# facebookresearch/AVID-CMA

Measured on AMD Instinct MI355X. Metric: clips/sec (video+audio fwd+bwd+NCE+Adam), higher is better.
Workload: dtype f32 (bf16x3 MFMA)

## Files before the change

### avid-cma_amd/avid_hip/lib.py

```python
from __future__ import annotations

import ctypes as C
import os
import subprocess


import torch

_HERE = os.path.dirname(os.path.abspath(__file__))
_PKG = os.path.dirname(_HERE)
LIB_PATH = os.environ.get("AVID_HIP_LIB") or os.path.join(_HERE, "libavid_hip.so")

AVID_OK = 0


class BnBwdFuse(C.Structure):
    _fields_ = [("x", C.c_void_p), ("scale", C.c_void_p), ("shift", C.c_void_p), ("mean", C.c_void_p),
                ("invstd", C.c_void_p), ("relu", C.c_int32), ("partials", C.c_void_p)]


class InAffine(C.Structure):
    _fields_ = [("scale", C.c_void_p), ("shift", C.c_void_p), ("relu", C.c_int32)]


# ... 79 lines not shown
    "avid_timing_enable": (_i, [_i]),
    "avid_timing_report": (_i, [C.c_char_p, _sz]),
    "avid_conv_fwd_workspace_bytes": (_sz, [_dp]),
    "avid_conv_fwd_stats_rows": (_i, [_dp]),
    "avid_conv_fwd": (_i, [_dp, _vp, _vp, _vp, _vp, _vp, _i, _vp, _vp, _vp, _sz, _vp]),
    "avid_conv_takes_in_affine": (_i, [_dp]),
    "avid_conv_fwd_in": (_i, [_dp, _vp, _vp, _vp, _vp, _vp, _vp, _i, _vp, _vp, _vp, _sz, _vp]),
    "avid_debug_in_affine_launches": (C.c_longlong, [_i]),
    "avid_conv_takes_out_affine": (_i, [_dp]),
    "avid_conv_fwd_out": (_i, [_dp, _vp, _vp, _vp, _vp, _vp, _vp, _i, _vp, _vp, _vp, _vp, _sz, _vp]),
    "avid_debug_out_affine_launches": (C.c_longlong, []),
    "avid_conv_dgrad_workspace_bytes": (_sz, [_dp]),
    "avid_conv_dgrad_bn_rows": (_i, [_dp]),
    "avid_conv_dgrad": (_i, [_dp, _vp, _vp, _vp, _vp, _vp, _vp, _vp, _vp, _vp, _sz, _vp]),
    "avid_weight_transpose_batched": (_i, [_i, _vp, _i64, _vp]),
    "avid_weight_transform": (_i, [_vp, _vp]),
    "avid_conv_wgrad_workspace_bytes": (_sz, [_dp]),
    "avid_conv_wgrad": (_i, [_dp, _vp, _vp, _vp, _vp, _sz, _vp]),
    "avid_conv_wgrad_in": (_i, [_dp, _vp, _vp, _vp, _vp, _vp, _sz, _vp]),
    "avid_conv_wgrad_groupable": (_i, [_dp]),
    "avid_conv_wgrad_group_workspace_bytes": (_sz, [_i, C.POINTER(WgradItem)]),
    "avid_conv_wgrad_group": (_i, [_i, C.POINTER(WgradItem), _vp, _sz, _vp]),
    "avid_conv_kernel_name": (_i, [_dp, _i, C.c_char_p, _i]),
    "avid_conv_uses_wino": (_i, [_dp, _i]),
    "avid_conv_uses_split": (_i, [_dp, _i]),
    "avid_conv_split_bytes": (_sz, [_dp]),
    "avid_debug_presplit_launches": (C.c_longlong, []),
    "avid_wino_configure": (_i, [_i, _i64, _i]),
    "avid_wino2_configure": (_i, [_i]),
    "avid_wino2_pre_configure": (_i, [_i]),
    "avid_wgrad_pre_configure": (_i, [_i]),
    "avid_stem_fwd_pre_configure": (_i, [_i]),
    "avid_tconv_configure": (_i, [_i]),
    "avid_set_cu_budget": (_i, [_i]),
    "avid_cu_budget": (_i, []),
    "avid_bn_workspace_bytes": (_sz, [_i64, _i]),
    "avid_bn_fwd_train": (_i, [_i64, _i, _vp, _vp, _vp, _vp, _vp, _f, _f, _i, _vp, _vp, _vp, _vp, _vp, _vp, _vp, _i, _vp, _sz, _vp]),
    "avid_bn_fwd_eval": (_i, [_i64, _i, _vp, _vp, _vp, _vp, _vp, _f, _i, _vp, _vp, _vp]),
    "avid_bn_eval_coeffs_batched": (_i, [_i, _vp, _vp]),
    "avid_bn_apply_eval": (_i, [_i64, _i, _vp, _vp, _vp, _i, _vp, _vp]),
    "avid_bn_relu_maxpool_fwd_eval": (_i, [_i, _i, _i, _i, _i, _vp, _vp, _vp, _vp, _vp]),
    "avid_bn_bwd": (_i, [_i64, _i, _vp, _vp, _vp, _vp, _vp, _vp, _vp, _i, _vp, _vp, _vp, _vp, _i, _i, _vp, _sz, _vp]),
    "avid_bn_relu_maxpool_fwd": (_i, [_i, _i, _i, _i, _i, _vp, _vp, _vp, _vp, _vp, _f, _f, _vp, _vp, _vp, _vp, _vp, _vp, _vp,
                                      _vp, _i, _vp, _sz, _vp]),
    "avid_bn_relu_maxpool_bwd": (_i, [_i, _i, _i, _i, _i, _vp, _vp, _vp, _vp, _vp, _vp, _vp, _vp, _vp, _vp, _vp, _vp, _sz,
                                      _vp]),
    "avid_clip_normalize": (_i, [_i, _i, _i, _i, _vp, C.POINTER(_f), C.POINTER(_f), _vp, _vp]),
    "avid_clip_augment_workspace_bytes": (_sz, [_i, C.POINTER(AugDesc), _i, _i, _i]),
    "avid_clip_augment": (_i, [_i, C.POINTER(AugDesc), _i, _i, _i, C.POINTER(_f), C.POINTER(_f), _vp, _vp, _sz, _vp]),
    "avid_logspec_basis_floats": (_sz, [_i]),
    "avid_logspec_basis": (_i, [_i, _vp, _vp]),
    "avid_logspec_workspace_bytes": (_sz, [_i, _i, _i]),
    "avid_logspec": (_i, [_i, _i, _vp, _i, _i, _i, _vp, _vp, _vp, _f, _vp, _vp, _sz, _vp]),
    "avid_maxpool_hw3s2_fwd": (_i, [_i, _i, _i, _i, _i, _vp, _vp, _vp, _vp]),
    "avid_maxpool_hw3s2_bwd": (_i, [_i, _i, _i, _i, _i, _vp, _vp, _vp, _vp]),
    "avid_global_maxpool_fwd": (_i, [_i, _i, _i, _vp, _vp, _vp, _vp]),
    "avid_global_maxpool_bwd": (_i, [_i, _i, _i, _vp, _vp, _vp, _vp]),
    "avid_relu_bwd": (_i, [_i64, _vp, _vp, _vp, _vp]),
    "avid_colsum": (_i, [_i64, _i, _vp, _vp, _vp]),
    "avid_l2norm_fwd": (_i, [_i, _i, _vp, _vp, _vp, _vp]),
    "avid_l2norm_bwd": (_i, [_i, _i, _vp, _vp, _vp, _vp, _vp]),
    "avid_alias_draw": (_i, [_i64, _i64, _vp, _vp, _i, _u64, _u64, _vp, _vp, _i64, _vp, _vp]),
    "avid_counter_add": (_i, [_vp, _u64, _vp]),
    "avid_dropout_fwd": (_i, [_i64, _i64, _f, _u64, _u64, _vp, _vp, _vp, _vp, _vp]),
    "avid_dropout_bwd": (_i, [_i64, _f, _vp, _vp, _vp, _vp]),
    "avid_cls_loss": (_i, [_i, _i, _i, _vp, _vp, _f, _vp, _vp, _vp, _vp, _vp, _vp]),
# ... 101 lines not shown
```

### avid-cma_amd/csrc/conv.hip

```cpp
#include <math.h>
#include <stdlib.h>

#include <atomic>
#include <type_traits>

#include "common.h"

namespace avid {

typedef unsigned int uintx4 __attribute__((ext_vector_type(4)));

struct ConvArgs {
  const float* __restrict__ src;
  const float* __restrict__ wk;
  int w_row, w_nrec;
  const float* __restrict__ addend;
  const float* __restrict__ bias;
  float* __restrict__ dst;
  float* __restrict__ part;
  int B, Ts, Hs, Ws, Cs;
  int Td, Hd, Wd, Cd;
  int kt, kh, kw;
  int st, sh, sw;
  int pt, ph, pw;
// ... 281 lines not shown

constexpr int EPI_ANY = 15;
#ifdef AVID_PK_TRACE
__device__ long long g_pk_trace[1024 * 64];
extern "C" int avid_debug_pk_trace(long long* host) {
  return (int)hipMemcpyFromSymbol(host, HIP_SYMBOL(g_pk_trace), sizeof(long long) * 1024 * 64);
}
#define PK_STAMP(idx) do { if (threadIdx.x == 0 && (idx) < 32) { g_pk_trace[blockIdx.x * 64 + (idx)] = wall_clock64(); g_pk_trace[blockIdx.x * 64 + 32 + (idx)] = clock64(); } } while (0)
#else
#define PK_STAMP(idx) do {} while (0)
#endif
#ifdef AVID_PK_FP32
constexpr bool PK_SPLIT = false;
#else
constexpr bool PK_SPLIT = true;
#endif
typedef __bf16 pk_bf16x8 __attribute__((ext_vector_type(8)));
typedef unsigned pk_uintx4 __attribute__((ext_vector_type(4)));
template <bool DOT = true>
__device__ __forceinline__ void pk_split8(const floatx4& v0, const floatx4& v1, pk_bf16x8& fh, pk_bf16x8& fm, pk_bf16x8& fl) {
  const float v[8] = {v0[0], v0[1], v0[2], v0[3], v1[0], v1[1], v1[2], v1[3]};
  unsigned h[4], m[4], l[4];
#pragma unroll
  for (int i = 0; i < 4; ++i) {
    if (DOT) split2_bf16_dot(v[2 * i], v[2 * i + 1], h[i], m[i], l[i]);
    else split2_bf16(v[2 * i], v[2 * i + 1], h[i], m[i], l[i]);
  }
  fh = __builtin_bit_cast(pk_bf16x8, pk_uintx4{h[0], h[1], h[2], h[3]});
  fm = __builtin_bit_cast(pk_bf16x8, pk_uintx4{m[0], m[1], m[2], m[3]});
  fl = __builtin_bit_cast(pk_bf16x8, pk_uintx4{l[0], l[1], l[2], l[3]});
}

constexpr int PK_BCH = 2 * 2 * 3 * 1024;
template <int WM, int WN, int TM, int TN, int MODE, bool STRIDED = false, int EPI = EPI_ANY, bool BS = false>
__global__ __launch_bounds__(WM * WN * 64, 2) void igemm_pk_kernel(const ConvArgs p) {
  static_assert(!STRIDED || MODE == 1, "parity classes are a dgrad construct");
  constexpr int NT = WM * WN * 64;
  constexpr int BM = WM * TM * 32, BN = WN * TN * 32;
  constexpr int RPP = NT / 8;
  constexpr int PA = BM / RPP, PB = BN / RPP;
  static_assert(BM % RPP == 0 && BN % RPP == 0, "tile rows must be a multiple of the staging pass");
  static_assert(!BS || (NT == 256 && (BN == 64 || BN == 128) && PK_SPLIT), "pre-split weights: the 4-wave tiles of the split-bf16 build");
  constexpr int BCH = (BN / 64) * PK_BCH;
  constexpr int PB3 = BCH / (NT * 16);
  constexpr bool ASWZ = BS && BN == 128;
  constexpr int ALD = ASWZ ? BK : LDK;
  constexpr int STAGE = BS ? BM * ALD + BCH / 4 : (BM + BN) * LDK;
  extern __shared__ __attribute__((aligned(16))) float smem[];
  typedef const ConvArgs __attribute__((address_space(4)))* KArgs;
  const KArgs kp = (KArgs)__builtin_amdgcn_kernarg_segment_ptr();
  const int tid = threadIdx.x, lane = tid & 63, wave = tid >> 6;
  const int wm = wave / WN, wn = wave % WN;
  const int lrow = tid >> 3, lcol = (tid & 7) * 4;
  const int h = lane >> 5, l31 = lane & 31;
  PK_STAMP(0);

  const int ntn = p.Cd / BN;
  const int G = gridDim.x;
  int slot_;
  if (p.pk_paired) {
    const int per = G >> 4;
    const int xcd = blockIdx.x & 7, pos = blockIdx.x >> 3;
    const int second = pos >= per ? 1 : 0;
    slot_ = second * (G >> 1) + xcd * per + (pos - second * per);
  } else {
    slot_ = (int)xcd_remap(blockIdx.x, G);
  }
  const int slot = __builtin_amdgcn_readfirstlane(slot_);
  const int ntaps = p.kt * p.kh * p.kw;
  const int cpt = p.Cs / BK;
  const int nk = ntaps * cpt;
  const int cs4 = p.Cs * 4;
  const int pix_per_b = p.Ts * p.Hs * p.Ws;
  const int pix_d = p.Td * p.Hd * p.Wd;
  const __amdgpu_buffer_rsrc_t rsB = __builtin_amdgcn_make_buffer_rsrc(
      BS ? const_cast<void*>(p.wsp) : (void*)p.wk, 0, BS ? p.wsp_nrec : p.w_nrec, 0x00020000);

  const int n_full = slot < p.pk_full ? (p.pk_full - slot + G - 1) / G : 0;
  int tslot = slot - p.pk_rot;
  tslot += tslot < 0 ? G : 0;
  const int nseg = n_full + (tslot < p.pk_tail_units ? 1 : 0);
// ... 49 lines not shown
      const int kps = (nkc + fc - 1) / fc;
      k0 = piece * kps < nkc ? piece * kps : nkc;
      k1 = k0 + kps < nkc ? k0 + kps : nkc;
      split = fc > 1 ? piece : -1;
    } else if (j < n_full) {
      tile = slot + j * G; k0 = 0; k1 = nk; split = -1;
    } else {
      int piece;
      if (p.pk_ws) {
        const int r = tslot / p.pk_ws, mt = tslot - r * p.pk_ws;
        const int nt = r / p.pk_f;
        piece = r - nt * p.pk_f;
        tile = p.pk_full + mt * ntn + nt;
      } else {
        tile = p.pk_full + tslot / p.pk_f;
        piece = tslot % p.pk_f;
      }
      split = p.pk_f > 1 ? piece : -1;
      k0 = piece * p.pk_kps;
      k1 = k0 + p.pk_kps < nk ? k0 + p.pk_kps : nk;
    }
  };

  int ld_seg = 0, ld_ks = 0, ld_kend = 0;
  int ld_dt = 0, ld_dh = 0, ld_dw = 0, ld_c0 = 0, ld_tap = 0;
  int ld_nh = p.kh, ld_nw = p.kw, ld_cls = 0;
  int ld_plo = 0, ld_phi = 0, ld_nrec = 0;
  int ld_soff_a = 0, ld_soff_b = 0;
  unsigned a_base[PA], a_mask[PA], a_cur[PA];
  unsigned b_off[PB];
  floatx4 va[PA], vb[PB];
  pk_uintx4 vb3[PB3];
  int ld_bnt = 0;

  auto range_mask = [](int lo, int hi, int k) -> unsigned {
    lo = lo < 0 ? 0 : lo;
    hi = hi > k - 1 ? k - 1 : hi;
    return hi >= lo ? (2u << hi) - (1u << lo) : 0u;
  };
  auto retap = [&]() {
    const int pixoff = ((ld_dt * p.Hs + ld_dh) * p.Ws + ld_dw) * cs4;
    const unsigned tap_off = (unsigned)(MODE == 0 ? pixoff : -pixoff);
    const unsigned sh_t = ld_dt, sh_h = 8 + ld_dh, sh_w = 16 + ld_dw;
#pragma unroll
    for (int i = 0; i < PA; ++i) {
      const unsigned okb = (a_mask[i] >> sh_t) & (a_mask[i] >> sh_h) & (a_mask[i] >> sh_w) & 1u;
      a_cur[i] = okb ? a_base[i] + tap_off : OOB;
    }
  };
  auto setup_tile = [&](int tile) {
    int c = 0, cT = p.Td, cH = p.Hd, cW = p.Wd, cM = p.M, cpix = pix_d, lt = tile;
    unsigned mgW = p.mgW, mgH = p.mgH, mgT = p.mgT;
    int shW = p.shW, shH = p.shH, shT = p.shT;
    int offt = p.pt, offh = p.ph, offw = p.pw, ndt = p.kt, ndh = p.kh, ndw = p.kw;
    if (STRIDED) {
      c = ld_cls;
      lt = tile - kp->cls_begin[c];
      cT = kp->cls_n[c][0]; cH = kp->cls_n[c][1]; cW = kp->cls_n[c][2];
      cpix = cT * cH * cW;
      cM = p.B * cpix;
      mgT = kp->cls_mg[c][0]; mgH = kp->cls_mg[c][1]; mgW = kp->cls_mg[c][2];
      shT = kp->cls_shf[c][0]; shH = kp->cls_shf[c][1]; shW = kp->cls_shf[c][2];
      offt = (kp->cls_p0[c][0] + p.pt - kp->cls_d0[c][0]) / p.st;
      offh = (kp->cls_p0[c][1] + p.ph - kp->cls_d0[c][1]) / p.sh;
      offw = (kp->cls_p0[c][2] + p.pw - kp->cls_d0[c][2]) / p.sw;
      ndt = kp->cls_nd[c][0]; ndh = kp->cls_nd[c][1]; ndw = kp->cls_nd[c][2];
// ... 33 lines not shown
        mh = range_mask(-h0, p.Hs - 1 - h0, p.kh);
        mw = range_mask(-w0, p.Ws - 1 - w0, p.kw);
      } else {
        t0 = td + offt; h0 = hd + offh; w0 = wd + offw;
        mt_ = range_mask(t0 - p.Ts + 1, t0, ndt);
        mh = range_mask(h0 - p.Hs + 1, h0, ndh);
        mw = range_mask(w0 - p.Ws + 1, w0, ndw);
      }
      dec_mask = ok ? (mt_ | (mh << 8) | (mw << 16)) : 0u;
      dec_base = (unsigned)((((b - b_lo) * p.Ts + t0) * p.Hs + h0) * p.Ws + w0) * cs4;
    }
#pragma unroll
    for (int i = 0; i < PA; ++i) {
      const int src = (lane & ~7) | i;
      a_mask[i] = (unsigned)__shfl((int)dec_mask, src, 64);
      a_base[i] = (unsigned)__shfl((int)dec_base, src, 64) + lcol * 4;
    }
#pragma unroll
    for (int i = 0; i < PB; ++i) b_off[i] = (unsigned)((n0 + lrow + RPP * i) * p.w_row + lcol) * 4;
    if (BS) ld_bnt = __builtin_amdgcn_readfirstlane(nt * BCH);
  };
  auto issue_loads = [&]() {
    const unsigned long long ptr = ((unsigned long long)(unsigned)__builtin_amdgcn_readfirstlane(ld_phi) << 32) |
                                   (unsigned)__builtin_amdgcn_readfirstlane(ld_plo);
    const __amdgpu_buffer_rsrc_t rsA = __builtin_amdgcn_make_buffer_rsrc(
        reinterpret_cast<void*>(ptr), 0, __builtin_amdgcn_readfirstlane(ld_nrec), 0x00020000);
    const int soff_a = __builtin_amdgcn_readfirstlane(ld_soff_a);
    const int soff_b = __builtin_amdgcn_readfirstlane(ld_soff_b);
#pragma unroll
    for (int i = 0; i < PA; ++i)
      va[i] = __builtin_bit_cast(floatx4, __builtin_amdgcn_raw_buffer_load_b128(rsA, a_cur[i], soff_a, 0));
    if (BS) {
      const int soff_b3 = __builtin_amdgcn_readfirstlane(ld_soff_b + ld_bnt);
#pragma unroll
      for (int i = 0; i < PB3; ++i)
        vb3[i] = __builtin_bit_cast(pk_uintx4, __builtin_amdgcn_raw_buffer_load_b128(rsB, (tid + NT * i) * 16, soff_b3, 0));
      return;
    }
#pragma unroll
    for (int i = 0; i < PB; ++i)
      vb[i] = __builtin_bit_cast(floatx4, __builtin_amdgcn_raw_buffer_load_b128(rsB, b_off[i], soff_b, 0));
  };
  const auto sgpr = [](int v) { return __builtin_amdgcn_readfirstlane(v); };
  auto set_tap = [&]() {
    if (STRIDED) {
      const int c = ld_cls;
      ld_tap = sgpr(((kp->cls_d0[c][0] + ld_dt * p.st) * p.kh + kp->cls_d0[c][1] + ld_dh * p.sh) * p.kw + kp->cls_d0[c][2] +
                    ld_dw * p.sw);
    } else {
      ld_tap = sgpr((ld_dt * p.kh + ld_dh) * p.kw + ld_dw);
    }
    ld_soff_a = sgpr(ld_c0 * 4);
    ld_soff_b = BS ? sgpr((ld_tap * cpt + ld_c0 / BK) * p.wsp_kstep) : sgpr((ld_tap * p.Cs + ld_c0) * 4);
  };
  auto setup_seg = [&](int j) {
    int tile, k0, k1, split;
    seg_info(j, tile, k0, k1, split);
    if (STRIDED) {
      while (k1 == k0 && j + 1 < nseg) seg_info(++j, tile, k0, k1, split);
      ld_seg = sgpr(k1 == k0 ? nseg : j);
      if (k1 == k0) return;
      ld_cls = sgpr(cls_of(tile));
      ld_nh = sgpr(kp->cls_nd[ld_cls][1]);
      ld_nw = sgpr(kp->cls_nd[ld_cls][2]);
    }
    ld_ks = sgpr(k0);
// ... 8 lines not shown
    setup_tile(tile);
  };
  auto advance = [&]() {
    ld_ks = sgpr(ld_ks + 1);
    ld_c0 = sgpr(ld_c0 + BK);
    bool moved = false;
    if (ld_ks == ld_kend) {
      ld_seg = sgpr(ld_seg + 1);
      if (ld_seg < nseg) {
        setup_seg(ld_seg);
        moved = ld_seg < nseg;
      }
    } else if (ld_c0 != p.Cs) {
      ld_soff_a = sgpr(ld_soff_a + BK * 4);
      ld_soff_b = sgpr(ld_soff_b + (BS ? p.wsp_kstep : BK * 4));
    } else {
      ld_c0 = 0;
      int dw = ld_dw + 1, dh = ld_dh, dt = ld_dt;
      if (dw == ld_nw) { dw = 0; ++dh; }
      if (dh == ld_nh) { dh = 0; ++dt; }
      ld_dw = sgpr(dw);
      ld_dh = sgpr(dh);
      ld_dt = sgpr(dt);
      set_tap();
      moved = true;
    }
    if (moved) retap();
  };
  auto store_stage = [&](float* st) {
#pragma unroll
    for (int i = 0; i < PA; ++i)
      *reinterpret_cast<floatx4*>(&st[(lrow + RPP * i) * ALD + (ASWZ ? (((tid & 7) ^ ((lrow >> 1) & 7)) << 2) : lcol)]) = va[i];
    if (BS) {
#pragma unroll
      for (int i = 0; i < PB3; ++i)
        *reinterpret_cast<pk_uintx4*>(reinterpret_cast<char*>(st + BM * ALD) + (tid + NT * i) * 16) = vb3[i];
      return;
    }
#pragma unroll
    for (int i = 0; i < PB; ++i) *reinterpret_cast<floatx4*>(&st[(BM + lrow + RPP * i) * LDK + lcol]) = vb[i];
  };

  setup_seg(0);
  if (!STRIDED || ld_seg < nseg) {
    retap();
    issue_loads();
    advance();
    store_stage(smem);
    if (ld_seg < nseg) {
      issue_loads();
      advance();
    }
  }
  __syncthreads();
  PK_STAMP(1);

  const int a_frag = (wm * TM * 32 + l31) * LDK + h * 4;
  const int b_frag = (BM + wn * TN * 32 + l31) * LDK + h * 4;
  int left = n_full * nk;
  if (STRIDED) {
    left = 0;
    for (int j = 0; j < nseg; ++j) {
      int tile, k0, k1, split;
      seg_info(j, tile, k0, k1, split);
      left += k1 - k0;
    }
  } else if (nseg > n_full) {
    int tile, k0, k1, split;
    seg_info(n_full, tile, k0, k1, split);
    left += k1 - k0;
  }
  int u = 0;
  floatx16 acc[TM][TN];

  auto ktile = [&](auto ST, auto LD) {
    const float* cur = smem + u * STAGE;
    float* nxt = smem + (u ^ 1) * STAGE;
    const float* Ab = cur + a_frag;
    const float* Bb = cur + b_frag;
    if (BS) {
      const float* As = ASWZ ? cur + (wm * TM * 32 + l31) * ALD : Ab - h * 4 + h * 8;
      const int akey = (l31 >> 1) & 7;
      const char* Bc = reinterpret_cast<const char*>(cur + BM * ALD) + lane * 16;
      floatx4 ar[2][TM][2];
      pk_bf16x8 bq[2][TN][3];
      auto fetch = [&](int st, int slot) {
        const int o0 = ASWZ ? (((st * 4 + h * 2) ^ akey) << 2) : st * 16;
        const int o1 = ASWZ ? (((st * 4 + h * 2 + 1) ^ akey) << 2) : st * 16 + 4;
#pragma unroll
        for (int i = 0; i < TM; ++i) {
          ar[slot][i][0] = *reinterpret_cast<const floatx4*>(As + i * 32 * ALD + o0);
          ar[slot][i][1] = *reinterpret_cast<const floatx4*>(As + i * 32 * ALD + o1);
        }
#pragma unroll
        for (int j = 0; j < TN; ++j) {
          const char* Bj = Bc + (((wn * TN + j) * 2 + st) * 3) * 1024;
          bq[slot][j][0] = *reinterpret_cast<const pk_bf16x8*>(Bj);
          bq[slot][j][1] = *reinterpret_cast<const pk_bf16x8*>(Bj + 1024);
          bq[slot][j][2] = *reinterpret_cast<const pk_bf16x8*>(Bj + 2048);
        }
      };
#ifdef AVID_PK_PREFETCH
      constexpr bool PF = TM * TN <= 2 && !STRIDED;
#else
      constexpr bool PF = false;
#endif
      fetch(0, 0);
#pragma unroll
      for (int st = 0; st < BK / 16; ++st) {
        if (PF) {
          if (st + 1 < BK / 16) fetch(st + 1, (st + 1) & 1);
          __builtin_amdgcn_sched_barrier(0);
        } else if (st > 0) {
          fetch(st, st & 1);
        }
        if (decltype(ST)::value && st == 0) store_stage(nxt);
// ... 81 lines not shown
          __builtin_amdgcn_sched_group_barrier(0x008, 1, 0);
          __builtin_amdgcn_sched_group_barrier(0x200, 1, 0);
        }
      }
      if (decltype(LD)::value && g == 1) {
#pragma unroll
        for (int q = 0; q < PA + PB; ++q) {
          __builtin_amdgcn_sched_group_barrier(0x008, 1, 0);
          __builtin_amdgcn_sched_group_barrier(0x020, 1, 0);
        }
      }
      __builtin_amdgcn_sched_barrier(0);
    }
  };

  const int row_bytes = p.Cd * 4;
  for (int j = 0; j < nseg; ++j) {
    int tile, k0, k1, split;
    seg_info(j, tile, k0, k1, split);
    const int nkj = k1 - k0;
#pragma unroll
    for (int i = 0; i < TM; ++i)
#pragma unroll
      for (int jj = 0; jj < TN; ++jj)
#pragma unroll
        for (int r = 0; r < 16; ++r) acc[i][jj][r] = 0.f;

    int nst = left - 2 < nkj ? left - 2 : nkj;
    if (nst < 0) nst = 0;
    PK_STAMP(2 + 3 * j);
    for (int ks = 0; ks < nst; ++ks, u ^= 1) {
      ktile(std::true_type{}, std::true_type{});
      advance();
      __syncthreads();
    }
    left -= nst;
    if (nst < nkj) {
      if (left == 2) {
        ktile(std::true_type{}, std::false_type{});
        __syncthreads();
        u ^= 1;
        --left;
        ++nst;
      }
      if (nst < nkj) {
        ktile(std::false_type{}, std::false_type{});
        __syncthreads();
        u ^= 1;
        --left;
      }
    }

    PK_STAMP(3 + 3 * j);
    if (STRIDED) {
      int* drow = reinterpret_cast<int*>(smem + 2 * STAGE);
      int* arow = drow + BM;
      const bool sparse_add = p.add_s[0] * p.add_s[1] * p.add_s[2] > 1;
      const int c = cls_of(tile);
      const int lt = tile - kp->cls_begin[c];
      const int mt = lt / ntn, nt = lt - mt * ntn;
      const int n0 = nt * BN;
      const int cT = kp->cls_n[c][0], cH = kp->cls_n[c][1], cW = kp->cls_n[c][2];
      __syncthreads();
      if (tid < BM) {
        const unsigned m = mt * BM + tid;
        const bool ok = m < (unsigned)(p.B * cT * cH * cW);
        const unsigned mm = ok ? m : 0u;
        const unsigned q1 = magic_div(mm, kp->cls_mg[c][2], kp->cls_shf[c][2]);
        const int wd = mm - q1 * cW;
        const unsigned q2 = magic_div(q1, kp->cls_mg[c][1], kp->cls_shf[c][1]);
        const int hd = q1 - q2 * cH;
        const int b = magic_div(q2, kp->cls_mg[c][0], kp->cls_shf[c][0]);
        const int td = q2 - b * cT;
        const int dst = ((b * p.Td + kp->cls_p0[c][0] + td * p.st) * p.Hd + kp->cls_p0[c][1] + hd * p.sh) * p.Wd +
                        kp->cls_p0[c][2] + wd * p.sw;
        drow[tid] = ok ? dst * row_bytes : (int)OOB;
        if (sparse_add) {
          const int t = kp->cls_p0[c][0] + td * p.st, hh = kp->cls_p0[c][1] + hd * p.sh, w = kp->cls_p0[c][2] + wd * p.sw;
          const bool on = ok && (t & (p.add_s[0] - 1)) == 0 && (hh & (p.add_s[1] - 1)) == 0 && (w & (p.add_s[2] - 1)) == 0;
          const int ar = ((b * p.add_n[0] + (t >> (p.add_s[0] - 1))) * p.add_n[1] + (hh >> (p.add_s[1] - 1))) * p.add_n[2] +
                         (w >> (p.add_s[2] - 1));
          arow[tid] = on ? ar * row_bytes : (int)OOB;
        } else {
          arow[tid] = ok ? dst * row_bytes : (int)OOB;
        }
      }
// ... 1812 lines not shown
  double best = 1e300;
  const int fmax = nk / 3 < 64 ? (nk / 3 < 1 ? 1 : nk / 3) : 64;
  for (long long m = T / C; m >= 0 && m >= T / C - 1; --m) {
    const long long full = m * C, tail = T - full;
    if (tail > G) continue;
    for (int f0 = 1; f0 <= (tail ? fmax : 1); ++f0) {
      const int kps = (nk + f0 - 1) / f0, f = (nk + kps - 1) / kps;
      const long long units = tail * f;
      if (units > G) break;
      const int maxu = units == 0 ? 0 : (int)((units + C - 1) / C);
      const double cost = (double)m * (nk + ovh) + (maxu == 2 ? 2.0 * pk_overlap() : (double)maxu) * (kps + ovh) + (f > 1 ? red : 0.0);
      if (cost < best - 1e-9) {
        best = cost;
        k.full = (int)full; k.tail_units = (int)units; k.f = f; k.kps = kps;
      }
    }
  }
  k.rot = per_cu == 2 ? (int)((k.full / C) % 2) * C : 0;
  k.tail_row0 = k.f > 1 ? (long long)(k.full / ntn) * k.BM : M;
  k.ws_floats = k.f > 1 ? (size_t)k.f * (size_t)(M - k.tail_row0) * Cd : 0;
  k.grid = G;
  k.paired = per_cu == 2 && G % 16 == 0;
  if ((long long)k.full + k.tail_units <= C / 2) {
    k.grid = k.full + k.tail_units;
    k.rot = 0;
    k.paired = false;
  }
  *cost_out = best * k.BN / 128.0;
  return k;
}

static PkPlan plan_pk(long long M, int Cd, int nk, int mode) {
  double c0, c1;
  if (Cd % 128 != 0) return plan_pk_tile(M, Cd, nk, 1, &c0, mode);
  const PkPlan wide = plan_pk_tile(M, Cd, nk, 0, &c0, mode);
  const PkPlan narrow = plan_pk_tile(M, Cd, nk, 1, &c1, mode);
  return c1 * 1.04 < c0 ? narrow : wide;
}

static int pk_ws_mode() {
  static std::atomic<int> v{-1};
  int m = v.load(std::memory_order_relaxed);
  if (m < 0) {
    const char* e = getenv("AVID_PK_WS");
    m = e ? atoi(e) : 1;
    if (m < 0 || m > 2) m = 1;
    v.store(m, std::memory_order_relaxed);
  }
  return m;
}
static int pk_slot_xcd(int slot, int G, bool paired) {
  if (paired) return (slot % (G >> 1)) / (G >> 4);
  if (G < 8) return slot;
  const int q = G / 8, r = G % 8;
  return slot < r * (q + 1) ? slot / (q + 1) : r + (slot - r * (q + 1)) / q;
}
static double pk_order_bytes(const PkPlan& pk, int ntn, int mtt, int nk, int cpt, double wbytes, bool ws) {
  if (mtt > 512 || ntn * pk.f > 1024) return 1e300;
  double total = 0.0;
  const int cb = cpt < 64 ? cpt : 64;
  for (int x = 0; x < 8; ++x) {
    bool wblk[1024] = {false};
    unsigned long long ablk[512] = {0};
    for (int u = 0; u < pk.tail_units; ++u) {
      if (pk_slot_xcd((u + pk.rot) % pk.grid, pk.grid, pk.paired) != x) continue;
      int mt, nt, piece;
// ... 77 lines not shown
}
constexpr int S2_WIDE_DEFAULT = 0;
static int bs_wide_mode() {
  static int v = -1;
  if (v < 0) {
    const char* e = getenv("AVID_BS_WIDE");
    v = e ? atoi(e) : 2;
    if (v < 0 || v > 2) v = 2;
  }
  return v;
}
static bool bs_rows() {
  static int v = -1;
  if (v < 0) {
    const char* e = getenv("AVID_BS_ROWS");
    v = e ? (atoi(e) != 0 ? 1 : 0) : 1;
  }
  return v != 0;
}
static bool s2_wide() {
  static std::atomic<int> v{-1};
  int m = v.load(std::memory_order_relaxed);
  if (m < 0) {
    const char* e = getenv("AVID_S2_WIDE");
    m = e ? (atoi(e) != 0 ? 1 : 0) : S2_WIDE_DEFAULT;
    v.store(m, std::memory_order_relaxed);
  }
  return m != 0;
}
static bool bs_wide(const PkPlan& pk) { return pk.tile == 0 && (bs_wide_mode() == 2 || (bs_wide_mode() == 1 && pk.full == 0)); }

static std::atomic<long long> g_presplit_launches{0};

template <int WM, int WN, int TM, int TN, int MODE, bool STRIDED, int EPI>
static void launch_pk_e(const ConvArgs& a, int grid, size_t lds, hipStream_t s) {
  if constexpr (pk_takes_split<WM, WN, TM, TN, EPI>() && !(STRIDED && WN == 2)) {
    if (a.wsp) {
      ++g_presplit_launches;
      constexpr int BM = WM * TM * 32, BN = WN * TN * 32;
      const size_t lds3 = sizeof(float) * 2 * (BM * (BN == 128 ? BK : LDK) + (BN / 64) * PK_BCH / 4) + (STRIDED ? sizeof(int) * 2 * BM : 0);
      launch_pk_eb<WM, WN, TM, TN, MODE, STRIDED, EPI, true>(a, grid, lds3, s);
      return;
    }
  }
  launch_pk_eb<WM, WN, TM, TN, MODE, STRIDED, EPI, false>(a, grid, lds, s);
}

template <int WM, int WN, int TM, int TN, int MODE, bool STRIDED = false>
static int launch_pk(const ConvArgs& a, int grid, hipStream_t s) {
  constexpr int BM = WM * TM * 32, BN = WN * TN * 32;
  const size_t lds = sizeof(float) * 2 * (BM + BN) * LDK + (STRIDED ? sizeof(int) * 2 * BM : 0);
  static char name[64] = "";
  if (!name[0]) snprintf(name, sizeof(name), "igemm_pk_kernel<%d,%d,%d,%d,%d>%s", WM, WN, TM, TN, MODE, STRIDED ? "s2" : "");
  const double K = (double)a.kt * a.kh * a.kw * a.Cs;
  const double srcpix = (double)a.B * a.Ts * a.Hs * a.Ws;
  const double flops = MODE == 1 ? 2.0 * srcpix * a.Cd * K : 2.0 * a.M * a.Cd * K;
  ScopedTimer t(s, name, flops,
                4.0 * (srcpix * a.Cs + (double)a.Cd * K + (double)a.M * a.Cd * (1 + (a.addend ? 1 : 0) + (a.bnb_x ? 1 : 0))));
  constexpr bool MAIN = (WM * WN == 4) || (WM == 2 && WN == 1);
  const int epi = MAIN ? epi_code<MODE>(a) : EPI_ANY;
  switch (epi) {
    case 0: launch_pk_e<WM, WN, TM, TN, MODE, STRIDED, MAIN ? 0 : EPI_ANY>(a, grid, lds, s); break;
    case 1: launch_pk_e<WM, WN, TM, TN, MODE, STRIDED, MAIN ? 1 : EPI_ANY>(a, grid, lds, s); break;
    case 2: launch_pk_e<WM, WN, TM, TN, MODE, STRIDED, (MAIN && MODE == 0 && !STRIDED) ? 2 : EPI_ANY>(a, grid, lds, s); break;
    case 3: launch_pk_e<WM, WN, TM, TN, MODE, STRIDED, (MAIN && MODE == 0 && !STRIDED) ? 3 : EPI_ANY>(a, grid, lds, s); break;
    case 4: launch_pk_e<WM, WN, TM, TN, MODE, STRIDED, (MAIN && MODE == 0 && !STRIDED) ? 4 : EPI_ANY>(a, grid, lds, s); break;
    case 5: launch_pk_e<WM, WN, TM, TN, MODE, STRIDED, (MAIN && MODE == 0 && !STRIDED) ? 5 : EPI_ANY>(a, grid, lds, s); break;
    case 8: launch_pk_e<WM, WN, TM, TN, MODE, STRIDED, (MAIN && MODE == 1) ? 8 : EPI_ANY>(a, grid, lds, s); break;
    case 9: launch_pk_e<WM, WN, TM, TN, MODE, STRIDED, (MAIN && MODE == 1) ? 9 : EPI_ANY>(a, grid, lds, s); break;
    default: launch_pk_e<WM, WN, TM, TN, MODE, STRIDED, EPI_ANY>(a, grid, lds, s); break;
  }
  return check_launch("igemm_pk");
// ... 471 lines not shown
  a.mgW = a.mgH = a.mgT = 0; a.shW = a.shH = a.shT = 0;
  a.add_s[0] = a.add_s[1] = a.add_s[2] = 1;
  a.add_n[0] = a.add_n[1] = a.add_n[2] = 0;
  a.wsp = nullptr;
  a.wsp_nrec = a.wsp_kstep = 0;
  a.stats_rows = 0;
  return dispatch_igemm<0>(a, nullptr, 0, s);
}

}

using namespace avid;

static bool conv_takes_split(const avid_conv_desc* d, int which) {
#ifdef AVID_NO_PRESPLIT
  return false;
#endif
  if (!PK_SPLIT || d->x_channel_first) return false;
  if (which == 0) {
    if (d->Cin % 32 || d->Cout % 64 || wino_supported(d, 0)) return false;
    const long long M = (long long)d->B * d->To * d->Ho * d->Wo;
    const PkPlan pk = plan_pk(M, d->Cout, trim_taps(d).d.kt * d->kh * d->kw * (d->Cin / BK), 0);
    return pk.tile == 1 || bs_wide(pk);
  }
  if (d->Cin % 64 || d->Cout % 32 || d->st > 2 || d->sh > 2 || d->sw > 2 || wino_supported(d, 1)) return false;
  const long long M = (long long)d->B * d->Ti * d->Hi * d->Wi;
  if (d->st > 1 || d->sh > 1 || d->sw > 1) return M * d->Cin * 4 < (1ll << 31) && (d->Cin % 128 != 0 || !s2_wide());
  const PkPlan pk = plan_pk(M, d->Cin, trim_taps(d).d.kt * d->kh * d->kw * (d->Cout / BK), 1);
  return pk.tile == 1 || bs_wide(pk);
}

extern "C" long long avid_debug_presplit_launches(void) { return g_presplit_launches.load(std::memory_order_relaxed); }

extern "C" int avid_tconv_configure(int mode) {
  g_tconv_mode.store((mode >= 0 && mode <= 2) ? mode : -1, std::memory_order_relaxed);
  return tconv_mode();
}

extern "C" int avid_conv_uses_split(const avid_conv_desc* d, int which) {
  if (!d || validate(d) || which < 0 || which > 1) return 0;
  return conv_takes_split(d, which) ? 1 : 0;
}

extern "C" size_t avid_conv_split_bytes(const avid_conv_desc* d) {
  if (!d || validate(d)) return 0;
  return (size_t)6 * d->Cout * d->kt * d->kh * d->kw * d->Cin;
}

static void set_split_operand(ConvArgs& a, const void* planes, int N, int C, int ntaps_full, int khw, int dt0) {
  const int kstep = (N / 64) * PK_BCH;
  const long long off = (long long)dt0 * khw * (C / BK) * kstep, total = (long long)ntaps_full * (C / BK) * kstep;
  a.wsp = static_cast<const char*>(planes) + off;
  a.wsp_nrec = (int)(total - off);
  a.wsp_kstep = kstep;
}

extern "C" size_t avid_conv_fwd_workspace_bytes(const avid_conv_desc* d) {
  if (!d || validate(d)) return 0;
  const bool vec = (d->Cin % 32 == 0) && !d->x_channel_first;
  if (!vec) return stem_fwd_supported(d) ? stem_fwd_ws_bytes(d) : 0;
  const long long M = (long long)d->B * d->To * d->Ho * d->Wo;
  const Trim tr = trim_taps(d);
  const int nk = tr.d.kt * d->kh * d->kw * (d->Cin / BK);
  size_t need = sizeof(float) * igemm_ws_floats(M, d->Cout, nk, 0);
  if (wino_supported(d, 0) && wino_ws_bytes(d, 0) > need) need = wino_ws_bytes(d, 0);
  return need;
// ... 747 lines not shown
```

### include/avid_hip.h

```cpp
#ifndef AVID_HIP_H
#define AVID_HIP_H

#include <stddef.h>
#include <stdint.h>

#ifdef __cplusplus
extern "C" {
#endif

#define AVID_OK 0
#define AVID_E_BADARG (-1)
#define AVID_E_SHAPE (-2)
#define AVID_E_HIP (-3)
#define AVID_E_UNSUPPORTED (-4)

typedef void* avid_stream_t;

const char* avid_last_error(void);
int avid_version(void);
int avid_device_info(int device, int* cu_count, int* lds_bytes, char* arch, int arch_len);

int avid_timing_enable(int on);
int avid_timing_report(char* buf, size_t len);

// ... 41 lines not shown
  const float* shift;
  const float* mean;
  const float* invstd;
  int32_t relu;
  float* partials;
} avid_bn_bwd_fuse;
int avid_conv_dgrad_bn_rows(const avid_conv_desc* d);
int avid_conv_dgrad(const avid_conv_desc* d, const float* dy, const float* w, const float* wt, const float* u,
                    const float* addend, const int32_t* addend_stride, float* dx, const avid_bn_bwd_fuse* bn,
                    void* ws, size_t ws_bytes, avid_stream_t stream);

typedef struct avid_wt_desc {
  const float* w;
  float* wt;
  int32_t Cout, ntaps, Cin;
  int32_t mode;
} avid_wt_desc;
int avid_weight_transpose_batched(int n, const avid_wt_desc* descs_dev, int64_t max_elems, avid_stream_t stream);
int avid_weight_transform(const avid_wt_desc* desc, avid_stream_t stream);

int avid_conv_kernel_name(const avid_conv_desc* d, int which, char* buf, int len);
int avid_conv_uses_wino(const avid_conv_desc* d, int which);
int avid_conv_uses_split(const avid_conv_desc* d, int which);
size_t avid_conv_split_bytes(const avid_conv_desc* d);
long long avid_debug_presplit_launches(void);

int avid_wino_configure(int enabled, int64_t min_pixels, int max_channels);
int avid_wino2_configure(int min_rounds_x10);
int avid_wino2_pre_configure(int on);
int avid_wgrad_pre_configure(int on);
int avid_stem_fwd_pre_configure(int on);

int avid_tconv_configure(int mode);

int avid_set_cu_budget(int cus);
int avid_cu_budget(void);

size_t avid_conv_wgrad_workspace_bytes(const avid_conv_desc* d);
int avid_conv_wgrad(const avid_conv_desc* d, const float* x, const float* dy, float* dw, void* ws,
                    size_t ws_bytes, avid_stream_t stream);
int avid_conv_wgrad_in(const avid_conv_desc* d, const float* x, const avid_in_affine* in, const float* dy, float* dw, void* ws,
                       size_t ws_bytes, avid_stream_t stream);

typedef struct avid_wgrad_item {
  avid_conv_desc d;
  const float* x;
  const float* dy;
  float* dw;
} avid_wgrad_item;
int avid_conv_wgrad_groupable(const avid_conv_desc* d);
size_t avid_conv_wgrad_group_workspace_bytes(int n, const avid_wgrad_item* items);
int avid_conv_wgrad_group(int n, const avid_wgrad_item* items, void* ws, size_t ws_bytes, avid_stream_t stream);

size_t avid_bn_workspace_bytes(int64_t M, int C);
int avid_bn_fwd_train(int64_t M, int C, const float* x, const float* gamma, const float* beta,
                      float* running_mean, float* running_var, float momentum, float eps, int relu,
                      float* y, float* save_mean, float* save_invstd, float* save_scale,
                      float* save_shift, int64_t* num_batches_tracked, const float* partials, int nparts,
                      void* ws, size_t ws_bytes, avid_stream_t stream);
int avid_bn_fwd_eval(int64_t M, int C, const float* x, const float* gamma, const float* beta,
                     const float* running_mean, const float* running_var, float eps, int relu,
                     float* y, float* save4, avid_stream_t stream);
typedef struct avid_bn_eval_item {
  const float* gamma;
  const float* beta;
  const float* running_mean;
// ... 233 lines not shown
```

Baseline: 6712.

## Stream pre-split weights into a 3-stage LDS ring via buffer-load-to-LDS DMA

For the 128x64 pre-split-weight implicit-GEMM tile, weight planes are now loaded straight into a static three-stage LDS ring with buffer_load...lds, skipping the register round trip. Per-k-tile __syncthreads are replaced by explicit vmcnt waits plus s_barrier. By default this only applies to strided (dgrad parity) launches. The aim is to cut register pressure and store instructions and to overlap weight fetch with MFMA work, at the cost of extra static LDS and delicate waitcnt accounting, especially around the epilogue.

```diff
diff --git a/avid-cma_amd/avid_hip/lib.py b/avid-cma_amd/avid_hip/lib.py
--- a/avid-cma_amd/avid_hip/lib.py
+++ b/avid-cma_amd/avid_hip/lib.py
@@ -135,6 +135,8 @@
     "avid_wgrad_pre_configure": (_i, [_i]),
     "avid_stem_fwd_pre_configure": (_i, [_i]),
     "avid_tconv_configure": (_i, [_i]),
+    "avid_pk_ring_configure": (_i, [_i]),
+    "avid_debug_pk_ring_launches": (C.c_longlong, []),
     "avid_set_cu_budget": (_i, [_i]),
     "avid_cu_budget": (_i, []),
     "avid_bn_workspace_bytes": (_sz, [_i64, _i]),
diff --git a/avid-cma_amd/csrc/conv.hip b/avid-cma_amd/csrc/conv.hip
--- a/avid-cma_amd/csrc/conv.hip
+++ b/avid-cma_amd/csrc/conv.hip
@@ -337,8 +337,20 @@
 }
 
 constexpr int PK_BCH = 2 * 2 * 3 * 1024;
-template <int WM, int WN, int TM, int TN, int MODE, bool STRIDED = false, int EPI = EPI_ANY, bool BS = false>
+typedef __attribute__((address_space(3))) void* pk_lds_ptr;
+__device__ __forceinline__ void pk_dma16(__amdgpu_buffer_rsrc_t rs, unsigned lds_addr, int voff, int soff) {
+  __builtin_amdgcn_raw_ptr_buffer_load_lds(rs, (pk_lds_ptr)(size_t)lds_addr, 16, voff, soff, 0, 0);
+}
+template <int VM>
+__device__ __forceinline__ void pk_wait_vm_lgkm0() {
+  static_assert(VM >= 0 && VM < 64, "vmcnt is a 6-bit field");
+  __builtin_amdgcn_s_waitcnt((VM & 15) | (7 << 4) | ((VM >> 4) << 14));
+}
+constexpr int PK_EPI_RING = 32;
+template <int WM, int WN, int TM, int TN, int MODE, bool STRIDED = false, int EPI_ = EPI_ANY, bool BS = false>
 __global__ __launch_bounds__(WM * WN * 64, 2) void igemm_pk_kernel(const ConvArgs p) {
+  constexpr int EPI = EPI_ & (PK_EPI_RING - 1);
+  constexpr bool RING = (EPI_ & PK_EPI_RING) != 0;
   static_assert(!STRIDED || MODE == 1, "parity classes are a dgrad construct");
   constexpr int NT = WM * WN * 64;
   constexpr int BM = WM * TM * 32, BN = WN * TN * 32;
@@ -350,8 +362,17 @@
   constexpr int PB3 = BCH / (NT * 16);
   constexpr bool ASWZ = BS && BN == 128;
   constexpr int ALD = ASWZ ? BK : LDK;
-  constexpr int STAGE = BS ? BM * ALD + BCH / 4 : (BM + BN) * LDK;
+  static_assert(!RING || (BS && BN == 64), "the weight ring is the 128 x 64 tile's (a third 24 KB stage costs the 128 x 128 tile its second workgroup)");
+  constexpr int STAGE = RING ? BM * ALD : (BS ? BM * ALD + BCH / 4 : (BM + BN) * LDK);
   extern __shared__ __attribute__((aligned(16))) float smem[];
+  constexpr int RING_STAGES = 3;
+  unsigned ring_lds = 0u;
+  const char* ring_b = nullptr;
+  if constexpr (RING) {
+    __shared__ __attribute__((aligned(16))) char ring_stages[RING_STAGES * BCH];
+    ring_lds = (unsigned)(size_t)(pk_lds_ptr)ring_stages;
+    ring_b = ring_stages;
+  }
   typedef const ConvArgs __attribute__((address_space(4)))* KArgs;
   const KArgs kp = (KArgs)__builtin_amdgcn_kernarg_segment_ptr();
   const int tid = threadIdx.x, lane = tid & 63, wave = tid >> 6;
@@ -467,6 +488,7 @@
   floatx4 va[PA], vb[PB];
   pk_uintx4 vb3[PB3];
   int ld_bnt = 0;
+  int ld_ring = 0, mm_ring = 0;
 
   auto range_mask = [](int lo, int hi, int k) -> unsigned {
     lo = lo < 0 ? 0 : lo;
@@ -566,6 +588,13 @@
       va[i] = __builtin_bit_cast(floatx4, __builtin_amdgcn_raw_buffer_load_b128(rsA, a_cur[i], soff_a, 0));
     if (BS) {
       const int soff_b3 = __builtin_amdgcn_readfirstlane(ld_soff_b + ld_bnt);
+      if (RING) {
+        const unsigned dst = __builtin_amdgcn_readfirstlane(ring_lds + ld_ring * BCH + wave * 1024);
+#pragma unroll
+        for (int i = 0; i < PB3; ++i) pk_dma16(rsB, dst + i * (NT * 16), (tid + NT * i) * 16, soff_b3);
+        ld_ring = __builtin_amdgcn_readfirstlane(ld_ring + 1 == RING_STAGES ? 0 : ld_ring + 1);
+        return;
+      }
 #pragma unroll
       for (int i = 0; i < PB3; ++i)
         vb3[i] = __builtin_bit_cast(pk_uintx4, __builtin_amdgcn_raw_buffer_load_b128(rsB, (tid + NT * i) * 16, soff_b3, 0));
@@ -640,6 +669,7 @@
     for (int i = 0; i < PA; ++i)
       *reinterpret_cast<floatx4*>(&st[(lrow + RPP * i) * ALD + (ASWZ ? (((tid & 7) ^ ((lrow >> 1) & 7)) << 2) : lcol)]) = va[i];
     if (BS) {
+      if (RING) return;
 #pragma unroll
       for (int i = 0; i < PB3; ++i)
         *reinterpret_cast<pk_uintx4*>(reinterpret_cast<char*>(st + BM * ALD) + (tid + NT * i) * 16) = vb3[i];
@@ -660,7 +690,7 @@
       advance();
     }
   }
-  __syncthreads();
+  if (!RING) __syncthreads();
   PK_STAMP(1);
 
   const int a_frag = (wm * TM * 32 + l31) * LDK + h * 4;
@@ -679,6 +709,7 @@
     left += k1 - k0;
   }
   int u = 0;
+  bool after_epi = false;
   floatx16 acc[TM][TN];
 
   auto ktile = [&](auto ST, auto LD) {
@@ -686,10 +717,17 @@
     float* nxt = smem + (u ^ 1) * STAGE;
     const float* Ab = cur + a_frag;
     const float* Bb = cur + b_frag;
+    if constexpr (RING) {
+      constexpr int N1 = decltype(ST)::value ? PA + PB3 : 0, NE = TM * TN * 16;
+      if (after_epi) pk_wait_vm_lgkm0<N1 + NE>(); else pk_wait_vm_lgkm0<N1>();
+      after_epi = false;
+      __builtin_amdgcn_s_barrier();
+    }
     if (BS) {
       const float* As = ASWZ ? cur + (wm * TM * 32 + l31) * ALD : Ab - h * 4 + h * 8;
       const int akey = (l31 >> 1) & 7;
-      const char* Bc = reinterpret_cast<const char*>(cur + BM * ALD) + lane * 16;
+      const char* Bc = RING ? ring_b + mm_ring * BCH + lane * 16 : reinterpret_cast<const char*>(cur + BM * ALD) + lane * 16;
+      if (RING) mm_ring = __builtin_amdgcn_readfirstlane(mm_ring + 1 == RING_STAGES ? 0 : mm_ring + 1);
       floatx4 ar[2][TM][2];
       pk_bf16x8 bq[2][TN][3];
       auto fetch = [&](int st, int slot) {
@@ -837,26 +875,27 @@
     for (int ks = 0; ks < nst; ++ks, u ^= 1) {
       ktile(std::true_type{}, std::true_type{});
       advance();
-      __syncthreads();
+      if (!RING) __syncthreads();
     }
     left -= nst;
     if (nst < nkj) {
       if (left == 2) {
         ktile(std::true_type{}, std::false_type{});
-        __syncthreads();
+        if (!RING) __syncthreads();
         u ^= 1;
         --left;
         ++nst;
       }
       if (nst < nkj) {
         ktile(std::false_type{}, std::false_type{});
-        __syncthreads();
+        if (!RING) __syncthreads();
         u ^= 1;
         --left;
       }
     }
 
     PK_STAMP(3 + 3 * j);
+    after_epi = true;
     if (STRIDED) {
       int* drow = reinterpret_cast<int*>(smem + 2 * STAGE);
       int* arow = drow + BM;
@@ -2735,6 +2774,7 @@
 
 static PkPlan plan_pk(long long M, int Cd, int nk, int mode) {
   double c0, c1;
+  if (Cd <= 0 || Cd % 64 != 0) return PkPlan{};
   if (Cd % 128 != 0) return plan_pk_tile(M, Cd, nk, 1, &c0, mode);
   const PkPlan wide = plan_pk_tile(M, Cd, nk, 0, &c0, mode);
   const PkPlan narrow = plan_pk_tile(M, Cd, nk, 1, &c1, mode);
@@ -2878,12 +2918,33 @@
 
 static std::atomic<long long> g_presplit_launches{0};
 
+constexpr int PK_RING_DEFAULT = 1;
+static std::atomic<int> g_pk_ring_mode{-1};
+static std::atomic<long long> g_pk_ring_launches{0};
+static int pk_ring_mode() {
+  int m = g_pk_ring_mode.load(std::memory_order_relaxed);
+  if (m < 0) {
+    const char* e = getenv("AVID_PK_RING");
+    m = e ? atoi(e) : PK_RING_DEFAULT;
+    if (m < 0 || m > 2) m = PK_RING_DEFAULT;
+    g_pk_ring_mode.store(m, std::memory_order_relaxed);
+  }
+  return m;
+}
+
 template <int WM, int WN, int TM, int TN, int MODE, bool STRIDED, int EPI>
 static void launch_pk_e(const ConvArgs& a, int grid, size_t lds, hipStream_t s) {
   if constexpr (pk_takes_split<WM, WN, TM, TN, EPI>() && !(STRIDED && WN == 2)) {
     if (a.wsp) {
       ++g_presplit_launches;
       constexpr int BM = WM * TM * 32, BN = WN * TN * 32;
+      if constexpr (BN == 64) {
+        if (pk_ring_mode() == 2 || (pk_ring_mode() == 1 && STRIDED)) {
+          ++g_pk_ring_launches;
+          launch_pk_eb<WM, WN, TM, TN, MODE, STRIDED, EPI | PK_EPI_RING, true>(a, grid, sizeof(float) * 2 * BM * LDK + (STRIDED ? sizeof(int) * 2 * BM : 0), s);
+          return;
+        }
+      }
       const size_t lds3 = sizeof(float) * 2 * (BM * (BN == 128 ? BK : LDK) + (BN / 64) * PK_BCH / 4) + (STRIDED ? sizeof(int) * 2 * BM : 0);
       launch_pk_eb<WM, WN, TM, TN, MODE, STRIDED, EPI, true>(a, grid, lds3, s);
       return;
@@ -3421,6 +3482,13 @@
 
 extern "C" long long avid_debug_presplit_launches(void) { return g_presplit_launches.load(std::memory_order_relaxed); }
 
+extern "C" long long avid_debug_pk_ring_launches(void) { return g_pk_ring_launches.load(std::memory_order_relaxed); }
+
+extern "C" int avid_pk_ring_configure(int mode) {
+  g_pk_ring_mode.store((mode >= 0 && mode <= 2) ? mode : -1, std::memory_order_relaxed);
+  return pk_ring_mode();
+}
+
 extern "C" int avid_tconv_configure(int mode) {
   g_tconv_mode.store((mode >= 0 && mode <= 2) ? mode : -1, std::memory_order_relaxed);
   return tconv_mode();
diff --git a/include/avid_hip.h b/include/avid_hip.h
--- a/include/avid_hip.h
+++ b/include/avid_hip.h
@@ -97,6 +97,9 @@
 int avid_stem_fwd_pre_configure(int on);
 
 int avid_tconv_configure(int mode);
+
+int avid_pk_ring_configure(int mode);
+long long avid_debug_pk_ring_launches(void);
 
 int avid_set_cu_budget(int cus);
 int avid_cu_budget(void);
```

Result: no change. 6710 (median of 2 runs) (-0.0%).
